# nsweb/dequan

Measured on NVIDIA B200. Metric: search_nodes_per_sec, higher is better.
Workload: dtype u32

## Files before the change

dequan_b200/csrc/dq_api.cu:

```cuda
#include <algorithm>
#include <condition_variable>
#include <cstdio>
#include <cstdlib>
#include <cstring>
#include <memory>
#include <mutex>
#include <string>
#include <thread>
#include <vector>

#include "dequan_b200.h"
#include "dq_kernels.cuh"
#include "dq_lane_queens.cuh"
#include "dq_lane_sudoku.cuh"
#include "dq_reg_graphs.cuh"
#include "dq_group_graphs.cuh"
#include "dq_small_tree.cuh"
#include "dq_lane_tree.cuh"
#include "dq_model.hpp"

namespace dq {

static thread_local std::string g_err;
void set_last_error(const std::string& s) { g_err = s; }
// ... 1135 lines not shown
}

static int run_batch_sudoku(dq_model* m, const uint8_t* cells_dev, int64_t n, int32_t stride, const dq_batch_opts* opts,
                            uint8_t* sol_dev, unsigned long long* nodes_dev, uint8_t* status_dev, dq_batch_stats* st) {
    int rc = DQ_OK;
    const unsigned long long task_cap = std::max<unsigned long long>(1u << 24, std::min<unsigned long long>(8ull * n, 1ull << 26));
    const unsigned long long snap_cap = std::min<unsigned long long>(std::max<unsigned long long>(1u << 20, (unsigned long long)n + (1u << 20)), 1ull << 24);
    const bool fresh_pool = m->s_tasks.cap < task_cap;
    DQ_CUDA(m->s_digest.reserve(n)); DQ_CUDA(m->s_hard.reserve(2 * (size_t)n)); DQ_CUDA(m->s_ctrl.reserve(16));
    DQ_CUDA(m->s_tasks.reserve(task_cap)); DQ_CUDA(m->s_snaps.reserve(snap_cap * kSnapWords)); DQ_CUDA(m->s_snap_state.reserve(snap_cap));
    unsigned long long* ctrl = m->s_ctrl.p;
    DQ_CUDA(cudaMemsetAsync(ctrl, 0, 16 * sizeof(unsigned long long), m->stream));
    DQ_CUDA(cudaMemsetAsync(m->s_snap_state.p, 0, snap_cap * sizeof(uint32_t), m->stream));
    const unsigned long long dirty = fresh_pool ? m->s_tasks.cap : std::min<unsigned long long>(m->s_tasks_used, m->s_tasks.cap);
    if (dirty) DQ_CUDA(cudaMemsetAsync(m->s_tasks.p, 0, dirty * sizeof(SudokuTask), m->stream));
    SudokuArgs A;
    A.digest = m->s_digest.p; A.n = n; A.stride = stride; A.cells = cells_dev; A.solution = sol_dev; A.nodes = nodes_dev;
    A.status = status_dev; A.hard = m->s_hard.p; A.tasks = m->s_tasks.p; A.task_cap = task_cap;
    A.snaps = m->s_snaps.p; A.snap_cap = snap_cap; A.snap_state = m->s_snap_state.p; A.ctrl = ctrl; A.user_budget = opts ? opts->node_budget : 0;
    A.force_donate = opts && opts->task_nodes > 0 ? (unsigned)opts->task_nodes : 0u;
    const char* env_dd = getenv("DQ_SUDOKU_DONATE_DEPTH");
    A.donate_depth = env_dd ? atoi(env_dd) : 5;
    const char* env_dm = getenv("DQ_SUDOKU_DONATE_MIN");
    const char* env_dg = getenv("DQ_SUDOKU_DONATE_GAP");
    A.donate_min = env_dm ? (unsigned)atoi(env_dm) : kDonateMinNodes;
    A.donate_gap = env_dg ? (unsigned)atoi(env_dg) : kDonateGap;
    const char* env_sg = getenv("DQ_SUDOKU_SPLIT_GAP");
    A.split_gap = env_sg ? (unsigned)atoi(env_sg) : kSplitGap;
    const char* env_h = getenv("DQ_SUDOKU_HIDDEN_AFTER");
    A.strong_hidden_after = env_h ? (unsigned)atoi(env_h) : kStrongHiddenAfter;
    const char* env_q = getenv("DQ_SUDOKU_POP_QUORUM");
    A.pop_quorum = env_q ? atoi(env_q) : kPopQuorum;
    const char* env_fb = getenv("DQ_SUDOKU_FIRST_BUDGET");
    A.first_budget = env_fb ? (unsigned)atoi(env_fb) : (n >= 400000 ? 3072u : 1024u);
    if (A.force_donate) A.first_budget = std::min(A.first_budget, 4u * A.force_donate);
    const bool trace = getenv("DQ_TRACE") != nullptr;
    cudaEvent_t ev[7] = {nullptr};
    if (trace) for (auto& e : ev) cudaEventCreate(&e);
    auto mark = [&](int i) { if (trace) cudaEventRecord(ev[i], m->stream); };
    const long long sms = m->sm_count;
    DQ_CUDA(cudaEventRecord(m->ev0, m->stream));
    mark(0);
    {
        int occ_d = 0;
        rc = max_ctas_per_sm(k_sudoku_digest, kDigestTile, kDigestSmem, &occ_d);
        if (rc != DQ_OK) return rc;
        const long long tiles = (n + kDigestTile - 1) / kDigestTile;
        k_sudoku_digest<<<(unsigned)std::max<long long>(1, std::min<long long>(tiles, (long long)std::max(occ_d, 1) * sms)), kDigestTile, kDigestSmem, m->stream>>>(
            cells_dev, n, stride, m->s_digest.p, ctrl + SKC_MAX_BLANK);
    }
    mark(1);
    unsigned long long* h_blank = m->pin + 117;
    DQ_CUDA(cudaMemcpyAsync(h_blank, ctrl + SKC_MAX_BLANK, sizeof(unsigned long long), cudaMemcpyDeviceToHost, m->stream));
    DQ_CUDA(cudaStreamSynchronize(m->stream));
    static const bool full_stack = getenv("DQ_SUDOKU_FULL_STACK") != nullptr;
    const int levels = full_stack ? 81 : (int)std::min<unsigned long long>(std::max<unsigned long long>(*h_blank, 1), 81);
    const size_t smem = offsetof(SudokuSmem, stk) + (size_t)levels * kSudokuBlock * sizeof(uint16_t);
    const size_t smem_strong = sudoku_strong_smem(levels);
    A.stack_levels = levels;
    int occ_first = 0, occ_count = 0, occ_walk = 0, occ_strong = 0;
    rc = max_ctas_per_sm(k_sudoku_first, kSudokuBlock, smem, &occ_first);
    if (rc == DQ_OK) rc = max_ctas_per_sm(k_sudoku_count, kSudokuBlock, smem, &occ_count);
    if (rc == DQ_OK) rc = max_ctas_per_sm(k_sudoku_walk, kSudokuBlock, smem, &occ_walk);
    if (rc == DQ_OK) rc = max_ctas_per_sm(k_sudoku_strong, 128, smem_strong, &occ_strong);
    if (rc != DQ_OK) return rc;
    if (occ_first < 1 || occ_count < 1 || occ_walk < 1 || occ_strong < 1) { g_err = "kernel does not fit an SM"; return DQ_ERR_UNSUPPORTED; }
    const long long ctas_first = std::max<long long>(1, std::min<long long>(occ_first * sms, (long long)((n + kSudokuBlock - 1) / kSudokuBlock)));
// ... 358 lines not shown
```

dequan_b200/csrc/dq_lane_sudoku.cuh:

```cuda
#pragma once
#include <cstdint>
#include <cuda_runtime.h>
#include "dq_group_graphs.cuh"

namespace dq {

constexpr int kSudokuBlock = 128;
constexpr uint32_t SK_ONES = 0x00100401u;
constexpr uint32_t SK_SPARE = 0x20080200u;
constexpr uint32_t SK_FULL3 = 0x1FF7FDFFu;
constexpr uint8_t SK_STATUS_HARD = 0xFD;
constexpr uint8_t SK_STATUS_DEFER = 0xFE;

constexpr int kDigestVec = 18;
constexpr int kTableWords = 63;
struct SudokuDigest { uint4 v[kDigestVec]; };

struct SudokuTask {
    uint32_t puzzle;
    uint32_t snap_id;
    uint32_t info;
    uint32_t pad;
};
constexpr uint32_t SKT_VALID = 0x80000000u, SKT_ROOT = 0x40000000u, SKT_NULL = 0x20000000u, SKT_TOP = 0x10000000u;
constexpr int kSnapWords = 12;

enum SkCtrl { SKC_FRESH = 0,
              SKC_HARD = 1,
              SKC_HARD_CUR = 2,
              SKC_WALK_CUR = 3,
              SKC_RESERVE = 4,
              SKC_SNAP = 5,
              SKC_HEAD = 6,
              SKC_OUTSTANDING = 7,
              SKC_MAX_BLANK = 8,
              SKC_ERROR = 9,
              SKC_TOTALS = 12 };

struct SudokuArgs {
    const SudokuDigest* digest;
    long long n;
    int stride;
    const uint8_t* cells;
    uint8_t* solution;
    unsigned long long* nodes;
    uint8_t* status;
    uint32_t* hard;
    SudokuTask* tasks;    unsigned long long task_cap;
    uint4* snaps;         unsigned long long snap_cap;
    uint32_t* snap_state;
    unsigned long long* ctrl;
    unsigned long long user_budget;
    unsigned first_budget;
    int donate_depth;
    unsigned donate_min, donate_gap;
    unsigned strong_hidden_after;
    int pop_quorum;
    int stack_levels;
    unsigned split_gap;
    unsigned force_donate;
};

constexpr int kDigestTile = 128;
constexpr int kDigestInBytes = kDigestTile * 81;
constexpr int kDigestOutBytes = kDigestTile * kDigestVec * 16;
constexpr int kDigestSmem = 2 * kDigestInBytes + kDigestOutBytes + 16;

__global__ void __launch_bounds__(kDigestTile)
k_sudoku_digest(const uint8_t* __restrict__ cells, long long n, int stride, SudokuDigest* __restrict__ out, unsigned long long* __restrict__ max_blank) {
    extern __shared__ __align__(128) uint8_t dg_raw[];
    uint8_t* recs = dg_raw + 2 * kDigestInBytes;
    const uint32_t in_s = smem_u32(dg_raw), recs_s = smem_u32(recs), mbar = recs_s + kDigestOutBytes;
    const long long tiles = (n + kDigestTile - 1) / kDigestTile;
    const bool bulk_ok = stride == 81 && ((size_t)cells & 15) == 0 && ((size_t)out & 15) == 0;
    if (threadIdx.x == 0) { mbar_init(mbar, 1); mbar_init(mbar + 8, 1); mbar_init_fence(); }
    __syncthreads();
    auto full = [&](long long t) { return bulk_ok && (t + 1) * kDigestTile <= n; };
    auto issue = [&](long long t, int b) {
        mbar_expect_tx(mbar + 8 * b, kDigestInBytes);
        bulk_g2s(in_s + b * kDigestInBytes, cells + t * kDigestInBytes, kDigestInBytes, mbar + 8 * b);
    };
    uint32_t parity = 0;
    int b = 0;
    int most_blanks = 0;
    long long t = blockIdx.x;
    if (t < tiles && full(t) && threadIdx.x == 0) issue(t, 0);
    bool store_in_flight = false;
    for (; t < tiles; t += gridDim.x, b ^= 1) {
        const long long nxt = t + gridDim.x;
        if (nxt < tiles && full(nxt) && threadIdx.x == 0) issue(nxt, b ^ 1);
        const long long first = t * kDigestTile;
        const int here = (int)min((long long)kDigestTile, n - first);
        uint8_t* stage = dg_raw + b * kDigestInBytes;
        if (full(t)) { mbar_wait(mbar + 8 * b, (parity >> b) & 1u); parity ^= 1u << b; }
// ... 6 lines not shown
            __syncthreads();
            store_in_flight = false;
        }
        if ((int)threadIdx.x < here) {
            const uint8_t* g = stage + threadIdx.x * 81;
            uint32_t row[9], col[9], box[9], blank[3] = {0, 0, 0};
#pragma unroll
            for (int i = 0; i < 9; i++) { row[i] = 0; col[i] = 0; box[i] = 0; }
            bool defer = false;
#pragma unroll
            for (int r = 0; r < 9; r++)
#pragma unroll
                for (int c = 0; c < 9; c++) {
                    const int p = r * 9 + c;
                    const uint32_t v = g[p];
                    if (v == 0) { blank[p >> 5] |= 1u << (p & 31); continue; }
                    if (v > 9) { defer = true; continue; }
                    const uint32_t bit = 1u << (v - 1);
                    const int bx = (r / 3) * 3 + c / 3;
                    if ((row[r] | col[c] | box[bx]) & bit) defer = true;
                    row[r] |= bit; col[c] |= bit; box[bx] |= bit;
                }
            uint32_t w[kDigestVec * 4];
#pragma unroll
            for (int i = 0; i < kDigestVec * 4; i++) w[i] = 0;
            int level = 0;
#pragma unroll
            for (int r = 0; r < 9; r++)
#pragma unroll
                for (int c = 0; c < 9; c++) {
                    const int p = r * 9 + c;
                    if (!((blank[p >> 5] >> (p & 31)) & 1u)) continue;
                    if ((row[r] | col[c] | box[(r / 3) * 3 + c / 3]) == 0x1FFu) defer = true;
                    w[19 + r * 3 + c / 3] |= 0x1FFu << (10 * (c % 3));
                    w[67 + (c * 9 + r) / 32] |= 1u << ((c * 9 + r) % 32);
                    ++level;
                }
            w[0] = blank[0]; w[1] = blank[1]; w[2] = blank[2];
            w[3] = (uint32_t)level | (defer ? 0x80000000u : 0u);
            most_blanks = max(most_blanks, level);
#pragma unroll
            for (int i = 0; i < 9; i++) w[10 + i] = box[i] * SK_ONES;
#pragma unroll
            for (int i = 0; i < 3; i++) {
                w[4 + i] = row[3 * i] | (row[3 * i + 1] << 10) | (row[3 * i + 2] << 20);
                w[7 + i] = col[3 * i] | (col[3 * i + 1] << 10) | (col[3 * i + 2] << 20);
            }
            uint32_t* rw = reinterpret_cast<uint32_t*>(recs + threadIdx.x * (kDigestVec * 16));
#pragma unroll
            for (int i = 0; i < kDigestVec * 4; i++) rw[i] = w[i];
            uint8_t* tab = recs + threadIdx.x * (kDigestVec * 16) + 46 * 4;
            int L = 0;
#pragma unroll
            for (int k = 0; k < 3; k++)
                for (uint32_t bits = blank[k]; bits; bits &= bits - 1u) tab[L++] = (uint8_t)(32 * k + __ffs((int)bits) - 1);
        }
        if (full(t)) {
            fence_async_smem();
            __syncthreads();
            if (threadIdx.x == 0) { bulk_s2g(out + first, recs_s, kDigestOutBytes); bulk_commit(); }
            store_in_flight = true;
        } else {
            __syncthreads();
            const uint4* src = reinterpret_cast<const uint4*>(recs);
            uint4* dst = reinterpret_cast<uint4*>(out + first);
            for (int i = threadIdx.x; i < here * kDigestVec; i += kDigestTile) dst[i] = src[i];
            __syncthreads();
        }
    }
    if (store_in_flight && threadIdx.x == 0) bulk_wait_read0();
    most_blanks = __reduce_max_sync(0xFFFFFFFFu, most_blanks);
    if ((threadIdx.x & 31) == 0 && most_blanks) atomicMax(max_blank, (unsigned long long)most_blanks);
}

struct SudokuSmem {
    uint32_t rowp[3][kSudokuBlock];
    uint32_t colp[3][kSudokuBlock];
    uint32_t boxr[9][kSudokuBlock];
    uint32_t blk[27][kSudokuBlock];
    uint32_t cellw[21][kSudokuBlock];
    uint16_t stk[81][kSudokuBlock];
};

__device__ __forceinline__ uint32_t sk_rep(uint32_t x9) { return x9 * SK_ONES; }

struct SkCell { int r, s, f, band, box, rm; };
__device__ __forceinline__ SkCell sk_decode(int p) {
    SkCell c;
    c.r = (p * 57) >> 9;
    const int col = p - 9 * c.r;
    c.s = (col * 11) >> 5;
    c.f = col - 3 * c.s;
    c.band = (c.r * 11) >> 5;
    c.box = c.band * 3 + c.s;
    c.rm = c.r - 3 * c.band;
    return c;
}

__device__ __forceinline__ uint32_t sk_singletons(uint32_t x) {
    const uint32_t y = x + (SK_SPARE - SK_ONES);
    const uint32_t z = x & y;
    const uint32_t tt = z + (SK_SPARE - SK_ONES);
    const uint32_t nz = ~tt & SK_SPARE;
    return x & (nz - (nz >> 9));
}

struct SkLane {
    bool have, enter;
    uint32_t puzzle;
    int p;
    SkCell c;
    int sp, base_sp, nblank;
    uint32_t passrem;
    uint32_t dom_rem;
    uint32_t nodes;
    unsigned long long nodes_hi;
};

__device__ __forceinline__ int sk_cell_at(const SudokuSmem& S, int t, int l) { return (int)((S.cellw[l >> 2][t] >> ((l & 3) * 8)) & 0xFF); }
__device__ __forceinline__ uint32_t sk_used_at(const SudokuSmem& S, int t, const SkCell& k) {
    return ((S.rowp[k.band][t] >> (10 * k.rm)) | (S.colp[k.s][t] >> (10 * k.f)) | S.boxr[k.box][t]) & 0x1FF;
}
__device__ __forceinline__ void sk_commit(SudokuSmem& S, int t, const SkCell& k, uint32_t bit) {
    S.rowp[k.band][t] |= bit << (10 * k.rm);
    S.boxr[k.box][t] |= sk_rep(bit);
    S.colp[k.s][t] |= bit << (10 * k.f);
}

__device__ __forceinline__ void sk_load_tables(SudokuSmem& S, int t, const uint4* __restrict__ dg) {
    uint32_t* dst = &S.rowp[0][t];
#pragma unroll
    for (int q = 1; q < kDigestVec; q++) {
        const uint4 x = __ldg(dg + q);
        const int wbase = 4 * q - 4;
        if (wbase + 0 < kTableWords) dst[(wbase + 0) * kSudokuBlock] = x.x;
        if (wbase + 1 < kTableWords) dst[(wbase + 1) * kSudokuBlock] = x.y;
        if (wbase + 2 < kTableWords) dst[(wbase + 2) * kSudokuBlock] = x.z;
        if (wbase + 3 < kTableWords) dst[(wbase + 3) * kSudokuBlock] = x.w;
    }
}
struct SkBlankT { uint32_t t0, t1, t2; };
__device__ __forceinline__ SkBlankT sk_load_blank_t(const uint4* __restrict__ dg) {
    const uint4 a = __ldg(dg + 16), b = __ldg(dg + 17);
    SkBlankT x; x.t0 = a.w; x.t1 = b.x; x.t2 = b.y;
    return x;
}

__device__ __forceinline__ void sk_enter(const SudokuSmem& S, int t, const SkCell& c, const SkBlankT& bt, uint32_t& dom, uint32_t& pass) {
    const uint32_t rowband = S.rowp[c.band][t];
    const uint32_t colw = S.colp[c.s][t];
    const uint32_t boxv = S.boxr[c.box][t];
    const uint32_t rowv = sk_rep((rowband >> (10 * c.rm)) & 0x1FF);
    const uint32_t colv = (colw >> (10 * c.f)) & 0x1FF;
    dom = ~(rowv | colv | boxv) & 0x1FF;
    uint32_t kill3 = sk_singletons(~(rowv | colw | boxv) & S.blk[c.r * 3 + c.s][t] & (0xFFFFFFFFu << (10 * c.f + 10)) & SK_FULL3);
    {
        const uint32_t* colp = &S.colp[c.s][t];
        const uint32_t* boxp = &S.boxr[c.box][t];
        const uint32_t* blkp = &S.blk[c.r * 3 + c.s][t];
#pragma unroll
        for (int k = 1; k <= 2; k++) {
            const bool on = c.s + k < 3;
            const uint32_t u = on ? (rowv | colp[k * kSudokuBlock] | boxp[k * kSudokuBlock]) : 0xFFFFFFFFu;
            const uint32_t b = on ? blkp[k * kSudokuBlock] : 0u;
            kill3 |= sk_singletons(~u & b);
        }
    }
    {
        const uint32_t* blkp = &S.blk[c.r * 3 + c.s][t];
#pragma unroll
        for (int k = 1; k <= 2; k++) {
            const bool on = c.rm + k < 3;
            const uint32_t rv = sk_rep((rowband >> (on ? 10 * (c.rm + k) : 0)) & 0x1FF);
            const uint32_t b = on ? blkp[3 * k * kSudokuBlock] : 0u;
            kill3 |= sk_singletons(~(rv | colw | boxv) & b);
        }
    }
    {
        const uint32_t crep = sk_rep(colv);
        const uint32_t* rowp = &S.rowp[c.band][t];
        const uint32_t* boxp = &S.boxr[c.box][t];
        const int q0 = 9 * (3 * c.s + c.f) + 3 * c.band;
#pragma unroll
        for (int k = 1; k <= 2; k++) {
            const bool on = c.band + k < 3;
            const int q = q0 + 3 * k;
            const uint32_t lo = q < 32 ? bt.t0 : (q < 64 ? bt.t1 : bt.t2);
            const uint32_t hi = q < 32 ? bt.t1 : (q < 64 ? bt.t2 : 0u);
            const uint32_t m3 = on ? (__funnelshift_r(lo, hi, q & 31) & 7u) : 0u;
            const uint32_t b = ((m3 * 0x00040201u) & SK_ONES) * 0x1FFu;
            const uint32_t u = on ? (crep | rowp[k * kSudokuBlock] | boxp[3 * k * kSudokuBlock]) : 0xFFFFFFFFu;
            kill3 |= sk_singletons(~u & b);
        }
    }
    const uint32_t kill = (kill3 | (kill3 >> 10) | (kill3 >> 20)) & 0x1FF;
    pass = dom & ~kill;
}

__device__ __forceinline__ bool sk_pop(SudokuSmem& S, int t, SkLane& L) {
    L.nodes += __popc(L.dom_rem);
    if (L.sp == L.base_sp) return true;
    --L.sp;
    const uint32_t e = S.stk[L.sp][t];
    const uint32_t v = e >> 9, bit = 1u << v;
    L.p = sk_cell_at(S, t, L.sp);
    L.c = sk_decode(L.p);
    S.rowp[L.c.band][t] ^= bit << (10 * L.c.rm);
    S.boxr[L.c.box][t] ^= sk_rep(bit);
    S.colp[L.c.s][t] ^= bit << (10 * L.c.f);
    L.passrem = e & 0x1FF;
    L.dom_rem = ~sk_used_at(S, t, L.c) & 0x1FF & ~((2u << v) - 1u);
    return false;
}

__device__ __forceinline__ bool sk_choose(SudokuSmem& S, int t, SkLane& L) {
    const uint32_t nxt = L.passrem & (0u - L.passrem);
    L.nodes += __popc(L.dom_rem & (nxt | (nxt - 1u)));
    L.passrem ^= nxt;
    const uint32_t v = __ffs(nxt) - 1;
    S.stk[L.sp][t] = (uint16_t)(L.passrem | (v << 9));
    if (L.sp == L.nblank - 1) return true;
    sk_commit(S, t, L.c, nxt);
    ++L.sp;
    L.p = sk_cell_at(S, t, L.sp);
    L.enter = true;
    return false;
}

__device__ __forceinline__ uint32_t sk_snap_entry(const uint4* __restrict__ sb, int l) {
    const uint4 cur = __ldcg(sb + (l >> 3));
    const uint32_t word = (l & 4) ? ((l & 2) ? cur.w : cur.z) : ((l & 2) ? cur.y : cur.x);
    return (l & 1) ? (word >> 16) : (word & 0xFFFF);
}
__device__ __forceinline__ void sk_snap_write(uint4* __restrict__ sb, const SudokuSmem& S, int t, int upto, uint32_t extra0, uint32_t extra1) {
    for (int q = 0; q * 8 <= upto + 1; q++) {
        uint32_t w4[4];
#pragma unroll
        for (int i = 0; i < 4; i++) {
            const int l0 = q * 8 + 2 * i, l1 = l0 + 1;
            const uint32_t e0 = l0 < upto ? (uint32_t)S.stk[l0][t] : (l0 == upto ? extra0 : (l0 == upto + 1 ? extra1 : 0u));
            const uint32_t e1 = l1 < upto ? (uint32_t)S.stk[l1][t] : (l1 == upto ? extra0 : (l1 == upto + 1 ? extra1 : 0u));
            w4[i] = e0 | (e1 << 16);
        }
        __stcg(sb + q, make_uint4(w4[0], w4[1], w4[2], w4[3]));
    }
}

constexpr int kPopQuorum = 10;

__device__ __forceinline__ void sk_store_solutions(const SudokuSmem& S, const SudokuArgs& A, int t, bool fin, uint32_t puzzle,
                                                   uint32_t b0, uint32_t b1, uint32_t b2) {
    const int lane = t & 31;
    const uint32_t lt = (1u << lane) - 1u;
    __syncwarp();
    uint32_t fm = __ballot_sync(0xFFFFFFFFu, fin);
    while (fm) {
        const int Ls = __ffs(fm) - 1;
        fm &= fm - 1;
        const uint32_t x0 = __shfl_sync(0xFFFFFFFFu, b0, Ls), x1 = __shfl_sync(0xFFFFFFFFu, b1, Ls), x2 = __shfl_sync(0xFFFFFFFFu, b2, Ls);
        const uint32_t pz = __shfl_sync(0xFFFFFFFFu, puzzle, Ls);
        uint8_t* out = A.solution + (size_t)pz * A.stride;
        const uint8_t* in = A.cells + (size_t)pz * A.stride;
        const int tL = (t & ~31) + Ls;
#pragma unroll
        for (int k = 0; k < 3; k++) {
            const int cell = lane + 32 * k;
            if (cell < 81) {
                const uint32_t bw = k == 0 ? x0 : (k == 1 ? x1 : x2);
                uint8_t val;
                if ((bw >> lane) & 1u) {
                    const int level = __popc(bw & lt) + (k > 0 ? __popc(x0) : 0) + (k > 1 ? __popc(x1) : 0);
                    val = (uint8_t)((S.stk[level][tL] >> 9) + 1);
                } else val = in[cell];
                out[cell] = val;
            }
        }
    }
}

__global__ void __launch_bounds__(kSudokuBlock)
k_sudoku_first(SudokuArgs A) {
    extern __shared__ __align__(16) unsigned char sk_raw[];
    SudokuSmem& S = *reinterpret_cast<SudokuSmem*>(sk_raw);
    const int t = threadIdx.x;
    const int lane = t & 31;
    const uint32_t lt = (1u << lane) - 1u;
    const unsigned long long total_warps = (unsigned long long)gridDim.x * (kSudokuBlock / 32);

    SkLane L = {};
    SkBlankT bt = {0, 0, 0};
    uint32_t b0 = 0, b1 = 0, b2 = 0;
    uint32_t limit = 0;
    bool limit_is_api = false, done = false;
    unsigned long long chunk_pos = 0, chunk_end = 0;
    bool exhausted = false;

    for (;;) {
        const uint32_t need = __ballot_sync(0xFFFFFFFFu, !L.have && !done);
        if (need) {
            const uint32_t n_need = __popc(need);
            if (chunk_pos >= chunk_end && !exhausted) {
                unsigned long long base = 0;
                uint32_t size = 0;
                if (lane == 0) {
                    const unsigned long long cur = *(volatile unsigned long long*)(A.ctrl + SKC_FRESH);
                    const unsigned long long remaining = cur < (unsigned long long)A.n ? (unsigned long long)A.n - cur : 0;
                    size = (uint32_t)min(max(remaining / (8ull * total_warps), (unsigned long long)n_need), 64ull);
                    base = atomicAdd(A.ctrl + SKC_FRESH, (unsigned long long)size);
                }
                base = __shfl_sync(0xFFFFFFFFu, base, 0);
                size = __shfl_sync(0xFFFFFFFFu, size, 0);
                chunk_pos = base;
                chunk_end = min(base + size, (unsigned long long)A.n);
                if (base >= (unsigned long long)A.n) { exhausted = true; chunk_end = chunk_pos; }
            }
            const unsigned long long avail = chunk_end - chunk_pos;
            if (!L.have && !done) {
                const uint32_t rank = __popc(need & lt);
                if (rank < avail) {
                    L.puzzle = (uint32_t)(chunk_pos + rank);
                    const uint4* dg = A.digest[L.puzzle].v;
                    const uint4 head = __ldg(dg);
                    b0 = head.x; b1 = head.y; b2 = head.z;
                    L.nblank = (int)(head.w & 0xFF);
                    L.nodes = 0; L.nodes_hi = 0;
                    limit = A.first_budget; limit_is_api = false;
                    bool skip = false;
                    if (head.w & 0x80000000u) { A.status[L.puzzle] = SK_STATUS_DEFER; skip = true; }
                    else if (A.user_budget) {
                        const unsigned long long givens = 81 - L.nblank;
                        if (A.user_budget < givens) {
                            A.nodes[L.puzzle] = A.user_budget + 1; A.status[L.puzzle] = 2; skip = true;
                            uint8_t* out = A.solution + (size_t)L.puzzle * A.stride;
                            for (int i = 0; i < 81; i++) out[i] = 0;
                        } else if (A.user_budget - givens + 1 <= (unsigned long long)limit) {
                            limit = (uint32_t)(A.user_budget - givens + 1);
                            limit_is_api = true;
                        }
                    }
                    if (!skip && L.nblank == 0) {
                        A.nodes[L.puzzle] = 81; A.status[L.puzzle] = 1;
                        uint8_t* out = A.solution + (size_t)L.puzzle * A.stride;
                        const uint8_t* in = A.cells + (size_t)L.puzzle * A.stride;
                        for (int i = 0; i < 81; i++) out[i] = in[i];
                        skip = true;
                    }
                    if (!skip) {
                        sk_load_tables(S, t, dg);
                        bt = sk_load_blank_t(dg);
                        L.sp = 0; L.base_sp = 0; L.passrem = 0; L.dom_rem = 0;
                        L.p = sk_cell_at(S, t, 0);
                        L.enter = true;
                        L.have = true;
                    }
                } else if (exhausted) done = true;
            }
            chunk_pos += min((unsigned long long)n_need, avail);
            if (__all_sync(0xFFFFFFFFu, done && !L.have)) break;
        }

        for (int rep = 0;; rep++) {
            const bool popping = L.have && !L.enter && L.passrem == 0;
            const uint32_t pm = __ballot_sync(0xFFFFFFFFu, popping);
            if (pm == 0 || (rep > 0 && __popc(pm) < A.pop_quorum)) break;
            if (popping && sk_pop(S, t, L)) {
                A.nodes[L.puzzle] = (81 - L.nblank) + L.nodes_hi + L.nodes;
                A.status[L.puzzle] = 0;
                uint8_t* out = A.solution + (size_t)L.puzzle * A.stride;
                for (int i = 0; i < 81; i++) out[i] = 0;
                L.have = false;
            }
        }

        bool fin = false;
        if (L.have && !L.enter && L.passrem != 0 && sk_choose(S, t, L)) {
            A.nodes[L.puzzle] = (81 - L.nblank) + L.nodes_hi + L.nodes;
            A.status[L.puzzle] = 1;
            fin = true;
            L.have = false;
        }

        if (L.have && L.enter) {
            L.c = sk_decode(L.p);
            uint32_t dom, pass;
            sk_enter(S, t, L.c, bt, dom, pass);
            L.dom_rem = dom; L.passrem = pass; L.enter = false;
        }

        if (L.have && L.nodes >= limit) {
            if (limit_is_api) {
                A.nodes[L.puzzle] = A.user_budget + 1; A.status[L.puzzle] = 2;
                uint8_t* out = A.solution + (size_t)L.puzzle * A.stride;
                for (int i = 0; i < 81; i++) out[i] = 0;
            } else {
                const unsigned long long sslot = atomicAdd(A.ctrl + SKC_SNAP, 1ull);
                const unsigned long long idx = atomicAdd(A.ctrl + SKC_HARD, 1ull);
                if (sslot < A.snap_cap) { sk_snap_write(A.snaps + (size_t)sslot * kSnapWords, S, t, L.sp, L.passrem, L.dom_rem); A.snap_state[sslot] = 1u; }
                else atomicOr(A.ctrl + SKC_ERROR, 2ull);
                A.hard[2 * idx] = L.puzzle;
                A.hard[2 * idx + 1] = (uint32_t)sslot | ((uint32_t)L.sp << 24);
                A.nodes[L.puzzle] = (81 - L.nblank) + L.nodes_hi + L.nodes;
                A.status[L.puzzle] = SK_STATUS_HARD;
            }
            L.have = false;
        }

        sk_store_solutions(S, A, t, fin, L.puzzle, b0, b1, b2);
    }
}

constexpr unsigned kStrongHiddenAfter = 400;

struct StrongSmem {
    uint32_t peer[81][32];
};
__host__ __device__ inline size_t sudoku_strong_smem(int levels) { return sizeof(StrongSmem) + (size_t)4 * levels * (32 * 4 + 2) + 16; }

__device__ __forceinline__ bool sk_hidden_singles(uint32_t& D, int lane, uint32_t u0, uint32_t u1, uint32_t u2, bool& changed) {
// ... 58 lines not shown
    uint16_t* const rest = reinterpret_cast<uint16_t*>(sk_raw + sizeof(StrongSmem) + (size_t)4 * A.stack_levels * 128) + wib * A.stack_levels;
    for (int i = threadIdx.x; i < 81 * 32; i += blockDim.x) {
        const int x = i >> 5, l = i & 31;
        const int xr = x / 9, xc = x % 9;
        uint32_t m = 0;
        for (int f = 0; f < 3; f++) {
            const int q = l + 32 * f;
            if (q >= 81 || q == x) continue;
            const int qr = q / 9, qc = q % 9;
            if (qr == xr || qc == xc || (qr / 3 == xr / 3 && qc / 3 == xc / 3)) m |= 1u << (10 * f);
        }
        M.peer[x][l] = m;
    }
    __syncthreads();
    const uint32_t valid3 = lane < 17 ? SK_ONES : 0x00000401u;
    uint32_t u0 = 0, u1 = 0, u2 = 0;
    if (lane < 27)
        for (int k = 0; k < 9; k++) {
            const int cell = lane < 9 ? lane * 9 + k : (lane < 18 ? k * 9 + (lane - 9)
                                                                  : ((lane - 18) / 3 * 3 + k / 3) * 9 + ((lane - 18) % 3 * 3 + k % 3));
            const uint32_t bit = 1u << (cell & 31);
            if (cell < 32) u0 |= bit; else if (cell < 64) u1 |= bit; else u2 |= bit;
        }
    const unsigned long long n_hard = A.ctrl[SKC_HARD];
    for (;;) {
        unsigned long long idx = 0;
        if (lane == 0) idx = atomicAdd(A.ctrl + SKC_HARD_CUR, 1ull);
        idx = __shfl_sync(0xFFFFFFFFu, idx, 0);
        if (idx >= n_hard) break;
        const uint32_t puzzle = A.hard[2 * idx];
        const uint8_t* in = A.cells + (size_t)puzzle * A.stride;
        const uint32_t* dw = reinterpret_cast<const uint32_t*>(A.digest[puzzle].v);
        const int nblank = (int)(__ldg(dw + 3) & 0xFF);
        const uint32_t cw = lane < 21 ? __ldg(dw + 46 + lane) : 0u;
        uint32_t D = 0;
#pragma unroll
        for (int f = 0; f < 3; f++) {
            const int q = lane + 32 * f;
            if (q < 81) {
                const uint32_t g = in[q];
                uint32_t field;
                if (g) field = (1u << (g - 1)) | 0x200u;
                else {
                    const SkCell k = sk_decode(q);
                    field = ~((__ldg(dw + 4 + k.band) >> (10 * k.rm)) | (__ldg(dw + 7 + k.s) >> (10 * k.f)) | __ldg(dw + 10 + k.box)) & 0x1FF;
                }
                D |= field << (10 * f);
            }
        }
        unsigned tries = 0;
        int l = sk_propagate(D, M, lane, valid3, false, u0, u1, u2) ? 0 : -1;
        bool back = false;
        while (l >= 0 && l < nblank) {
            const int p = (int)((__shfl_sync(0xFFFFFFFFu, cw, l >> 2) >> ((l & 3) * 8)) & 0xFF);
            const int owner = p & 31, f = p >> 5;
            uint32_t d;
            if (!back) {
                const uint32_t w = __shfl_sync(0xFFFFFFFFu, D, owner) >> (10 * f);
                if (w & 0x200u) {
                    if (lane == 0) rest[l] = 0;
                    __syncwarp();
                    ++l;
                    continue;
                }
                d = w & 0x1FF;
                saved[l * 32] = D;
            } else d = rest[l];
            bool ok = false;
            while (d) {
                const uint32_t v = d & (0u - d);
                d ^= v;
                D = saved[l * 32];
                if (lane == owner) D = (D & ~(0x3FFu << (10 * f))) | ((v | 0x200u) << (10 * f));
                D &= ~(M.peer[p][lane] * v);
                ++tries;
                if (sk_propagate(D, M, lane, valid3, tries > A.strong_hidden_after, u0, u1, u2)) { ok = true; break; }
            }
            __syncwarp();
            if (lane == 0) rest[l] = (uint16_t)d;
            __syncwarp();
            if (ok) { ++l; back = false; }
            else {
                --l;
                while (l >= 0 && rest[l] == 0) --l;
                back = true;
            }
        }
// ... 5 lines not shown
            if (q < 81) out[q] = sat ? (uint8_t)__ffs((D >> (10 * f)) & 0x1FF) : (uint8_t)0;
        }
        if (lane == 0) A.status[puzzle] = sat ? 1 : 0;
        __syncwarp();
    }
}

__global__ void __launch_bounds__(kSudokuBlock)
k_sudoku_walk(SudokuArgs A) {
    extern __shared__ __align__(16) unsigned char sk_raw[];
    SudokuSmem& S = *reinterpret_cast<SudokuSmem*>(sk_raw);
    const int t = threadIdx.x;
    const int lane = t & 31;
    const unsigned long long n_hard = A.ctrl[SKC_HARD];
    auto emit = [&](uint32_t puzzle, uint32_t snap, uint32_t info) {
        const unsigned long long slot = atomicAdd(A.ctrl + SKC_RESERVE, 1ull);
        if (slot >= A.task_cap) { atomicOr(A.ctrl + SKC_ERROR, 2ull); return; }
        atomicAdd(A.ctrl + SKC_OUTSTANDING, 1ull);
        *reinterpret_cast<uint4*>(A.tasks + slot) = make_uint4(puzzle, snap, SKT_VALID | info, 0u);
    };
    for (;;) {
        unsigned long long base = 0;
        if (lane == 0) base = atomicAdd(A.ctrl + SKC_WALK_CUR, 32ull);
        base = __shfl_sync(0xFFFFFFFFu, base, 0);
        if (base >= n_hard) break;
        const bool active = base + lane < n_hard;
        const uint32_t puzzle = active ? A.hard[2 * (base + lane)] : 0u;
        const uint32_t hinfo = active ? A.hard[2 * (base + lane) + 1] : 0u;
        const uint32_t snap = hinfo & 0xFFFFFFu;
        const int psp = (int)(hinfo >> 24);
        const uint4* sb = A.snaps + (size_t)snap * kSnapWords;
        int nblank = 0;
        bool sat = false;
        SkBlankT bt = {0, 0, 0};
        if (active) {
            const uint4* dg = A.digest[puzzle].v;
            nblank = (int)(__ldg(dg).w & 0xFF);
            sk_load_tables(S, t, dg);
            bt = sk_load_blank_t(dg);
            sat = A.status[puzzle] == 1;
        }
        const uint8_t* sol = A.solution + (size_t)puzzle * A.stride;
        if (active && !sat) emit(puzzle, snap, SKT_TOP | 0u | ((uint32_t)psp << 8));
        unsigned long long direct = 0;
        bool on_parked_path = true;
        const int levels = active && sat ? nblank : 0;
        const int max_levels = __reduce_max_sync(0xFFFFFFFFu, levels);
        for (int l = 0; l < max_levels; l++) {
            if (l < levels) {
                const int p = sk_cell_at(S, t, l);
                const SkCell c = sk_decode(p);
                const uint32_t bit = 1u << (sol[p] - 1);
                uint32_t dom_rem, passrem;
                bool charge = true;
                if (on_parked_path && l < psp) {
                    const uint32_t e = sk_snap_entry(sb, l);
                    const uint32_t v = e >> 9;
                    if ((1u << v) == bit) charge = false;
                    else {
                        if ((1u << v) > bit) atomicOr(A.ctrl + SKC_ERROR, 8ull);
                        emit(puzzle, snap, SKT_TOP | (uint32_t)(l + 1) | ((uint32_t)psp << 8));
                        passrem = e & 0x1FF;
                        dom_rem = ~sk_used_at(S, t, c) & 0x1FF & ~((2u << v) - 1u);
                        on_parked_path = false;
                    }
                } else if (on_parked_path && l == psp) {
                    passrem = sk_snap_entry(sb, l) & 0x1FF;
                    dom_rem = sk_snap_entry(sb, l + 1) & 0x1FF;
                    on_parked_path = false;
                } else {
                    uint32_t dom, pass;
                    sk_enter(S, t, c, bt, dom, pass);
                    dom_rem = dom; passrem = pass;
                }
                if (charge) {
                    direct += __popc(dom_rem & (bit | (bit - 1u)));
                    if (!(passrem & bit)) atomicOr(A.ctrl + SKC_ERROR, 8ull);
                    uint32_t V = passrem & (bit - 1u);
                    while (V) {
                        const uint32_t v = __ffs(V) - 1;
                        V &= V - 1;
                        emit(puzzle, 0u, SKT_ROOT | (uint32_t)l | (v << 8));
                    }
                }
                sk_commit(S, t, c, bit);
            }
        }
        if (active && direct) atomicAdd(A.nodes + puzzle, direct);
    }
}

constexpr int kDonatePeriod = 32;
constexpr uint32_t kDonateMinNodes = 48;
constexpr uint32_t kDonateGap = 96;
constexpr uint32_t kSplitGap = 512;

__global__ void __launch_bounds__(kSudokuBlock)
k_sudoku_count(SudokuArgs A) {
    extern __shared__ __align__(16) unsigned char sk_raw[];
    SudokuSmem& S = *reinterpret_cast<SudokuSmem*>(sk_raw);
    const int t = threadIdx.x;
    const int lane = t & 31;
    const uint32_t lt = (1u << lane) - 1u;
    const unsigned long long total_warps = (unsigned long long)gridDim.x * (kSudokuBlock / 32);
    volatile unsigned long long* vctrl = A.ctrl;

    SkLane L = {};
    SkBlankT bt = {0, 0, 0};
    uint32_t donate_at = 0;
    uint32_t split_at = 0;
    bool waiting = false, poll_now = false;
    unsigned long long ticket = 0;
    int iter = 0;
    unsigned spins = 0;

    for (;;) {
        {
            const uint32_t need = __ballot_sync(0xFFFFFFFFu, !L.have && !waiting);
            if (need) {
                unsigned long long base = 0;
                if (lane == 0) base = atomicAdd(A.ctrl + SKC_HEAD, (unsigned long long)__popc(need));
                base = __shfl_sync(0xFFFFFFFFu, base, 0);
                if (!L.have && !waiting) { ticket = base + __popc(need & lt); waiting = true; poll_now = true; }
            }
        }
        unsigned closed_now = 0;
        uint32_t got_info = 0, got_snap = 0;
        if (waiting && (poll_now || (iter & 7) == 0) && ticket < A.task_cap) {
            volatile uint32_t* rec = reinterpret_cast<volatile uint32_t*>(A.tasks + ticket);
            const uint32_t info = rec[2];
            if (info) {
                __threadfence();
                waiting = false;
                L.puzzle = rec[0];
                if (info & SKT_NULL) closed_now = 1;
                else { got_info = info; got_snap = rec[1]; }
            }
        }
        for (uint32_t todo = __ballot_sync(0xFFFFFFFFu, got_info != 0u); todo; todo &= todo - 1u) {
            const int src = __ffs((int)todo) - 1;
            const uint32_t pz = __shfl_sync(0xFFFFFFFFu, L.puzzle, src), inf = __shfl_sync(0xFFFFFFFFu, got_info, src);
            const uint32_t sn = __shfl_sync(0xFFFFFFFFu, got_snap, src);
            const int ts = (t & ~31) + src;
            const uint32_t* dgw = reinterpret_cast<const uint32_t*>(A.digest[pz].v);
            uint32_t* tab = &S.rowp[0][0];
            for (int w = lane; w < kTableWords; w += 32) tab[w * kSudokuBlock + ts] = __ldg(dgw + 4 + w);
            __syncwarp();
            const bool root = (inf & SKT_ROOT) != 0u;
            const int lo = (int)(inf & 0xFF), hi = (int)((inf >> 8) & 0xFF);
            const int n_replay = root ? lo + 1 : hi;
            const uint8_t* sol = A.solution + (size_t)pz * A.stride;
            const uint4* sb = A.snaps + (size_t)sn * kSnapWords;
            for (int l = lane; l < n_replay; l += 32) {
                const int q = sk_cell_at(S, ts, l);
                uint32_t v, entry;
                if (root) { v = l < lo ? (uint32_t)sol[q] - 1u : (uint32_t)(hi & 0xF); entry = v << 9; }
                else { const uint32_t e = sk_snap_entry(sb, l); v = e >> 9; entry = l >= lo ? e : (e & 0xFE00u); }
                const SkCell k = sk_decode(q);
                const uint32_t bit = 1u << v;
                atomicOr(&S.rowp[k.band][ts], bit << (10 * k.rm));
                atomicOr(&S.boxr[k.box][ts], sk_rep(bit));
                atomicOr(&S.colp[k.s][ts], bit << (10 * k.f));
                S.stk[l][ts] = (uint16_t)entry;
            }
            __syncwarp();
        }
        if (got_info) {
            const uint32_t info = got_info;
            const uint4* dg = A.digest[L.puzzle].v;
            L.nblank = (int)(__ldg(dg).w & 0xFF);
            bt = sk_load_blank_t(dg);
            L.nodes = 0; L.nodes_hi = 0;
            L.passrem = 0; L.dom_rem = 0;
            L.have = true;
            donate_at = A.force_donate ? A.force_donate : A.donate_min;
            split_at = A.split_gap;
            if (info & SKT_ROOT) {
                const int l0 = (int)(info & 0xFF);
                L.sp = l0 + 1; L.base_sp = l0 + 1;
                if (L.sp >= L.nblank) { atomicOr(A.ctrl + SKC_ERROR, 4ull); L.have = false; closed_now = 1; }
                else { L.p = sk_cell_at(S, t, L.sp); L.enter = true; }
            } else {
                const int lo = (int)(info & 0xFF), hi = (int)((info >> 8) & 0xFF);
                const uint4* sb = A.snaps + (size_t)got_snap * kSnapWords;
                L.sp = hi; L.base_sp = lo;
                L.p = sk_cell_at(S, t, hi);
                L.c = sk_decode(L.p);
                const uint32_t e = sk_snap_entry(sb, hi);
                L.passrem = e & 0x1FF;
                if (info & SKT_TOP) L.dom_rem = sk_snap_entry(sb, hi + 1) & 0x1FF;
                else L.dom_rem = ~sk_used_at(S, t, L.c) & 0x1FF & ~((2u << (e >> 9)) - 1u);
                L.enter = false;
                __threadfence();
                A.snap_state[got_snap] = 0u;
            }
        }
        poll_now = false;
        {
            const uint32_t cm = __ballot_sync(0xFFFFFFFFu, closed_now != 0);
            if (cm && lane == 0) atomicAdd(A.ctrl + SKC_OUTSTANDING, 0ull - (unsigned long long)__popc(cm));
            if (cm) continue;
        }
        if (__ballot_sync(0xFFFFFFFFu, L.have) == 0) {
            unsigned long long out = 0;
            if (lane == 0) out = vctrl[SKC_OUTSTANDING];
            out = __shfl_sync(0xFFFFFFFFu, out, 0);
            if (out == 0) break;
            __nanosleep(spins < 4096u ? 200u : 2000u);
            if (++spins > 120000000u) { if (lane == 0) atomicOr(A.ctrl + SKC_ERROR, 1ull); break; }
            poll_now = true;
            continue;
        }
        spins = 0;
        ++iter;

        if ((iter & (kDonatePeriod - 1)) == 0) {
            long long demand = 0;
            if (lane == 0) {
                const unsigned long long h = vctrl[SKC_HEAD], r = vctrl[SKC_RESERVE];
                demand = h > r ? (long long)(h - r) : 0;
// ... 22 lines not shown
                            atomicAdd(A.ctrl + SKC_OUTSTANDING, 0ull - 1ull);
                            A.snap_state[sslot] = 0u;
                            donate_at = 0xFFFFFFFFu; split_at = 0xFFFFFFFFu;
                        } else {
                            sk_snap_write(A.snaps + (size_t)sslot * kSnapWords, S, t, hl + 1, 0u, 0u);
                            volatile uint32_t* rec = reinterpret_cast<volatile uint32_t*>(A.tasks + slot);
                            rec[0] = L.puzzle; rec[1] = (uint32_t)sslot;
                            __threadfence();
                            rec[2] = SKT_VALID | (uint32_t)L.base_sp | ((uint32_t)hl << 8);
                            L.base_sp = hl + 1;
                            donate_at = L.nodes + (A.force_donate ? A.force_donate : A.donate_gap);
                            split_at = L.nodes + A.split_gap;
                        }
                    }
                }
            }
        }

        unsigned closed = 0;
        for (int rep = 0;; rep++) {
            const bool popping = L.have && !L.enter && L.passrem == 0;
            const uint32_t pm = __ballot_sync(0xFFFFFFFFu, popping);
            if (pm == 0 || (rep > 0 && __popc(pm) < A.pop_quorum)) break;
            if (popping && sk_pop(S, t, L)) {
                atomicAdd(A.nodes + L.puzzle, L.nodes_hi + L.nodes);
                L.have = false; closed = 1;
            }
        }

        if (L.have && !L.enter && L.passrem != 0 && sk_choose(S, t, L))
            atomicOr(A.ctrl + SKC_ERROR, 4ull);

        if (L.have && L.enter) {
            L.c = sk_decode(L.p);
            uint32_t dom, pass;
            sk_enter(S, t, L.c, bt, dom, pass);
            L.dom_rem = dom; L.passrem = pass; L.enter = false;
        }
        if (L.nodes >= 0x80000000u) { L.nodes_hi += L.nodes; L.nodes = 0; donate_at = 0; split_at = A.split_gap; }

        {
            const uint32_t cm = __ballot_sync(0xFFFFFFFFu, closed != 0);
            if (cm && lane == 0) atomicAdd(A.ctrl + SKC_OUTSTANDING, 0ull - (unsigned long long)__popc(cm));
        }
    }
}

__global__ void k_sudoku_finish(SudokuArgs A, unsigned long long* totals) {
    const long long i = (long long)blockIdx.x * blockDim.x + threadIdx.x;
    unsigned sat = 0, unsat = 0, budget = 0;
    unsigned long long nd = 0;
    if (i < A.n) {
        uint8_t st = A.status[i];
        if (st != SK_STATUS_DEFER) {
            if (A.user_budget && A.nodes[i] > A.user_budget && st != 2) {
                st = 2;
                A.nodes[i] = A.user_budget + 1;
                uint8_t* out = A.solution + (size_t)i * A.stride;
                for (int c = 0; c < 81; c++) out[c] = 0;
            }
            A.status[i] = st;
            nd = A.nodes[i];
            sat = st == 1; unsat = st == 0; budget = st == 2;
        }
    }
    for (int o = 16; o > 0; o >>= 1) {
        sat += __shfl_down_sync(0xFFFFFFFFu, sat, o);
        unsat += __shfl_down_sync(0xFFFFFFFFu, unsat, o);
        budget += __shfl_down_sync(0xFFFFFFFFu, budget, o);
// ... 18 lines not shown
```

Baseline: 565.1 billion.

## Compact sudoku digest: replace per-cell blank masks with bit masks and packed cell descriptors

Shrinks the per-puzzle digest from 18 to 12 uint4 words. The 27 shared-memory blank-mask words are replaced by compact row-major and column-major blank bitmaps kept in registers, and the cell order table now stores pre-decoded band/row/stack/column descriptors instead of raw cell indices. This removes the sk_decode arithmetic, a large block of shared memory per thread, and digest bandwidth, which should raise occupancy and lower memory traffic. The cost is some extra shift and select logic in sk_enter. The first-task node budget for large batches is also lowered from 3072 to 2048.

```diff
diff --git a/dequan_b200/csrc/dq_api.cu b/dequan_b200/csrc/dq_api.cu
--- a/dequan_b200/csrc/dq_api.cu
+++ b/dequan_b200/csrc/dq_api.cu
@@ -1191,7 +1191,7 @@
     const char* env_q = getenv("DQ_SUDOKU_POP_QUORUM");
     A.pop_quorum = env_q ? atoi(env_q) : kPopQuorum;
     const char* env_fb = getenv("DQ_SUDOKU_FIRST_BUDGET");
-    A.first_budget = env_fb ? (unsigned)atoi(env_fb) : (n >= 400000 ? 3072u : 1024u);
+    A.first_budget = env_fb ? (unsigned)atoi(env_fb) : (n >= 400000 ? 2048u : 1024u);
     if (A.force_donate) A.first_budget = std::min(A.first_budget, 4u * A.force_donate);
     const bool trace = getenv("DQ_TRACE") != nullptr;
     cudaEvent_t ev[7] = {nullptr};
diff --git a/dequan_b200/csrc/dq_lane_sudoku.cuh b/dequan_b200/csrc/dq_lane_sudoku.cuh
--- a/dequan_b200/csrc/dq_lane_sudoku.cuh
+++ b/dequan_b200/csrc/dq_lane_sudoku.cuh
@@ -12,8 +12,8 @@
 constexpr uint8_t SK_STATUS_HARD = 0xFD;
 constexpr uint8_t SK_STATUS_DEFER = 0xFE;
 
-constexpr int kDigestVec = 18;
-constexpr int kTableWords = 63;
+constexpr int kDigestVec = 12;
+constexpr int kTableWords = 36;
 struct SudokuDigest { uint4 v[kDigestVec]; };
 
 struct SudokuTask {
@@ -60,6 +60,30 @@
     unsigned split_gap;
     unsigned force_donate;
 };
+
+struct SkCell { int s, f, band, box, rm; };
+__host__ __device__ __forceinline__ SkCell sk_decode(int p) {
+    SkCell c;
+    const int r = (p * 57) >> 9;
+    const int col = p - 9 * r;
+    c.s = (col * 11) >> 5;
+    c.f = col - 3 * c.s;
+    c.band = (r * 11) >> 5;
+    c.box = c.band * 3 + c.s;
+    c.rm = r - 3 * c.band;
+    return c;
+}
+__host__ __device__ __forceinline__ uint32_t sk_desc(int p) {
+    const SkCell c = sk_decode(p);
+    return (uint32_t)(c.band | c.rm << 2 | c.s << 4 | c.f << 6);
+}
+__device__ __forceinline__ SkCell sk_unpack(uint32_t d) {
+    SkCell c;
+    c.band = d & 3; c.rm = (d >> 2) & 3; c.s = (d >> 4) & 3; c.f = d >> 6;
+    c.box = c.band * 3 + c.s;
+    return c;
+}
+__device__ __forceinline__ int sk_desc_cell(uint32_t d) { return 27 * (d & 3) + 9 * ((d >> 2) & 3) + 3 * ((d >> 4) & 3) + (d >> 6); }
 
 constexpr int kDigestTile = 128;
 constexpr int kDigestInBytes = kDigestTile * 81;
@@ -132,8 +156,8 @@
                     const int p = r * 9 + c;
                     if (!((blank[p >> 5] >> (p & 31)) & 1u)) continue;
                     if ((row[r] | col[c] | box[(r / 3) * 3 + c / 3]) == 0x1FFu) defer = true;
-                    w[19 + r * 3 + c / 3] |= 0x1FFu << (10 * (c % 3));
-                    w[67 + (c * 9 + r) / 32] |= 1u << ((c * 9 + r) % 32);
+                    w[40 + r / 3] |= 1u << (10 * (c % 3) + 3 * (r % 3) + c / 3);
+                    w[44 + c / 3] |= 1u << (10 * (r % 3) + 3 * (c % 3) + r / 3);
                     ++level;
                 }
             w[0] = blank[0]; w[1] = blank[1]; w[2] = blank[2];
@@ -149,11 +173,11 @@
             uint32_t* rw = reinterpret_cast<uint32_t*>(recs + threadIdx.x * (kDigestVec * 16));
 #pragma unroll
             for (int i = 0; i < kDigestVec * 4; i++) rw[i] = w[i];
-            uint8_t* tab = recs + threadIdx.x * (kDigestVec * 16) + 46 * 4;
+            uint8_t* tab = recs + threadIdx.x * (kDigestVec * 16) + 19 * 4;
             int L = 0;
 #pragma unroll
             for (int k = 0; k < 3; k++)
-                for (uint32_t bits = blank[k]; bits; bits &= bits - 1u) tab[L++] = (uint8_t)(32 * k + __ffs((int)bits) - 1);
+                for (uint32_t bits = blank[k]; bits; bits &= bits - 1u) tab[L++] = (uint8_t)sk_desc(32 * k + __ffs((int)bits) - 1);
         }
         if (full(t)) {
             fence_async_smem();
@@ -177,25 +201,11 @@
     uint32_t rowp[3][kSudokuBlock];
     uint32_t colp[3][kSudokuBlock];
     uint32_t boxr[9][kSudokuBlock];
-    uint32_t blk[27][kSudokuBlock];
-    uint32_t cellw[21][kSudokuBlock];
+    uint32_t lvl[21][kSudokuBlock];
     uint16_t stk[81][kSudokuBlock];
 };
 
 __device__ __forceinline__ uint32_t sk_rep(uint32_t x9) { return x9 * SK_ONES; }
-
-struct SkCell { int r, s, f, band, box, rm; };
-__device__ __forceinline__ SkCell sk_decode(int p) {
-    SkCell c;
-    c.r = (p * 57) >> 9;
-    const int col = p - 9 * c.r;
-    c.s = (col * 11) >> 5;
-    c.f = col - 3 * c.s;
-    c.band = (c.r * 11) >> 5;
-    c.box = c.band * 3 + c.s;
-    c.rm = c.r - 3 * c.band;
-    return c;
-}
 
 __device__ __forceinline__ uint32_t sk_singletons(uint32_t x) {
     const uint32_t y = x + (SK_SPARE - SK_ONES);
@@ -205,10 +215,17 @@
     return x & (nz - (nz >> 9));
 }
 
+__device__ __forceinline__ uint32_t sk_singletons_at(uint32_t x, uint32_t blank) {
+    const uint32_t y = x + (SK_SPARE - SK_ONES);
+    const uint32_t z = x & y;
+    const uint32_t tt = z + (SK_SPARE - SK_ONES);
+    const uint32_t one = ~(tt >> 9) & blank & SK_ONES;
+    return x & (one * 0x1FFu);
+}
+
 struct SkLane {
     bool have, enter;
     uint32_t puzzle;
-    int p;
     SkCell c;
     int sp, base_sp, nblank;
     uint32_t passrem;
@@ -217,7 +234,7 @@
     unsigned long long nodes_hi;
 };
 
-__device__ __forceinline__ int sk_cell_at(const SudokuSmem& S, int t, int l) { return (int)((S.cellw[l >> 2][t] >> ((l & 3) * 8)) & 0xFF); }
+__device__ __forceinline__ uint32_t sk_desc_at(const SudokuSmem& S, int t, int l) { return (S.lvl[l >> 2][t] >> ((l & 3) * 8)) & 0xFF; }
 __device__ __forceinline__ uint32_t sk_used_at(const SudokuSmem& S, int t, const SkCell& k) {
     return ((S.rowp[k.band][t] >> (10 * k.rm)) | (S.colp[k.s][t] >> (10 * k.f)) | S.boxr[k.box][t]) & 0x1FF;
 }
@@ -239,58 +256,51 @@
         if (wbase + 3 < kTableWords) dst[(wbase + 3) * kSudokuBlock] = x.w;
     }
 }
-struct SkBlankT { uint32_t t0, t1, t2; };
-__device__ __forceinline__ SkBlankT sk_load_blank_t(const uint4* __restrict__ dg) {
-    const uint4 a = __ldg(dg + 16), b = __ldg(dg + 17);
-    SkBlankT x; x.t0 = a.w; x.t1 = b.x; x.t2 = b.y;
+struct SkBlank { uint32_t w0, w1, w2, t0, t1, t2; };
+__device__ __forceinline__ SkBlank sk_load_blank(const uint4* __restrict__ dg) {
+    const uint4 a = __ldg(dg + 10), b = __ldg(dg + 11);
+    SkBlank x; x.w0 = a.x; x.w1 = a.y; x.w2 = a.z; x.t0 = b.x; x.t1 = b.y; x.t2 = b.z;
     return x;
 }
 
-__device__ __forceinline__ void sk_enter(const SudokuSmem& S, int t, const SkCell& c, const SkBlankT& bt, uint32_t& dom, uint32_t& pass) {
+__device__ __forceinline__ void sk_enter(const SudokuSmem& S, int t, const SkCell& c, const SkBlank& bl, uint32_t& dom, uint32_t& pass) {
     const uint32_t rowband = S.rowp[c.band][t];
     const uint32_t colw = S.colp[c.s][t];
     const uint32_t boxv = S.boxr[c.box][t];
     const uint32_t rowv = sk_rep((rowband >> (10 * c.rm)) & 0x1FF);
     const uint32_t colv = (colw >> (10 * c.f)) & 0x1FF;
     dom = ~(rowv | colv | boxv) & 0x1FF;
-    uint32_t kill3 = sk_singletons(~(rowv | colw | boxv) & S.blk[c.r * 3 + c.s][t] & (0xFFFFFFFFu << (10 * c.f + 10)) & SK_FULL3);
+    const uint32_t xb = (c.band == 0 ? bl.w0 : (c.band == 1 ? bl.w1 : bl.w2)) >> (3 * c.rm + c.s);
+    uint32_t kill3 = sk_singletons_at(~(rowv | colw | boxv) & (0xFFFFFFFFu << (10 * c.f + 10)) & SK_FULL3, xb);
     {
         const uint32_t* colp = &S.colp[c.s][t];
         const uint32_t* boxp = &S.boxr[c.box][t];
-        const uint32_t* blkp = &S.blk[c.r * 3 + c.s][t];
 #pragma unroll
         for (int k = 1; k <= 2; k++) {
             const bool on = c.s + k < 3;
             const uint32_t u = on ? (rowv | colp[k * kSudokuBlock] | boxp[k * kSudokuBlock]) : 0xFFFFFFFFu;
-            const uint32_t b = on ? blkp[k * kSudokuBlock] : 0u;
-            kill3 |= sk_singletons(~u & b);
+            kill3 |= sk_singletons_at(~u & SK_FULL3, xb >> k);
         }
     }
     {
-        const uint32_t* blkp = &S.blk[c.r * 3 + c.s][t];
 #pragma unroll
         for (int k = 1; k <= 2; k++) {
             const bool on = c.rm + k < 3;
             const uint32_t rv = sk_rep((rowband >> (on ? 10 * (c.rm + k) : 0)) & 0x1FF);
-            const uint32_t b = on ? blkp[3 * k * kSudokuBlock] : 0u;
-            kill3 |= sk_singletons(~(rv | colw | boxv) & b);
+            const uint32_t u = on ? (rv | colw | boxv) : 0xFFFFFFFFu;
+            kill3 |= sk_singletons_at(~u & SK_FULL3, xb >> (3 * k));
         }
     }
     {
         const uint32_t crep = sk_rep(colv);
         const uint32_t* rowp = &S.rowp[c.band][t];
         const uint32_t* boxp = &S.boxr[c.box][t];
-        const int q0 = 9 * (3 * c.s + c.f) + 3 * c.band;
+        const uint32_t xs = (c.s == 0 ? bl.t0 : (c.s == 1 ? bl.t1 : bl.t2)) >> (3 * c.f + c.band);
 #pragma unroll
         for (int k = 1; k <= 2; k++) {
             const bool on = c.band + k < 3;
-            const int q = q0 + 3 * k;
-            const uint32_t lo = q < 32 ? bt.t0 : (q < 64 ? bt.t1 : bt.t2);
-            const uint32_t hi = q < 32 ? bt.t1 : (q < 64 ? bt.t2 : 0u);
-            const uint32_t m3 = on ? (__funnelshift_r(lo, hi, q & 31) & 7u) : 0u;
-            const uint32_t b = ((m3 * 0x00040201u) & SK_ONES) * 0x1FFu;
             const uint32_t u = on ? (crep | rowp[k * kSudokuBlock] | boxp[3 * k * kSudokuBlock]) : 0xFFFFFFFFu;
-            kill3 |= sk_singletons(~u & b);
+            kill3 |= sk_singletons_at(~u & SK_FULL3, xs >> k);
         }
     }
     const uint32_t kill = (kill3 | (kill3 >> 10) | (kill3 >> 20)) & 0x1FF;
@@ -303,8 +313,7 @@
     --L.sp;
     const uint32_t e = S.stk[L.sp][t];
     const uint32_t v = e >> 9, bit = 1u << v;
-    L.p = sk_cell_at(S, t, L.sp);
-    L.c = sk_decode(L.p);
+    L.c = sk_unpack(sk_desc_at(S, t, L.sp));
     S.rowp[L.c.band][t] ^= bit << (10 * L.c.rm);
     S.boxr[L.c.box][t] ^= sk_rep(bit);
     S.colp[L.c.s][t] ^= bit << (10 * L.c.f);
@@ -322,7 +331,7 @@
     if (L.sp == L.nblank - 1) return true;
     sk_commit(S, t, L.c, nxt);
     ++L.sp;
-    L.p = sk_cell_at(S, t, L.sp);
+    L.c = sk_unpack(sk_desc_at(S, t, L.sp));
     L.enter = true;
     return false;
 }
@@ -388,7 +397,7 @@
     const unsigned long long total_warps = (unsigned long long)gridDim.x * (kSudokuBlock / 32);
 
     SkLane L = {};
-    SkBlankT bt = {0, 0, 0};
+    SkBlank bl = {0, 0, 0, 0, 0, 0};
     uint32_t b0 = 0, b1 = 0, b2 = 0;
     uint32_t limit = 0;
     bool limit_is_api = false, done = false;
@@ -447,9 +456,9 @@
                     }
                     if (!skip) {
                         sk_load_tables(S, t, dg);
-                        bt = sk_load_blank_t(dg);
+                        bl = sk_load_blank(dg);
                         L.sp = 0; L.base_sp = 0; L.passrem = 0; L.dom_rem = 0;
-                        L.p = sk_cell_at(S, t, 0);
+                        L.c = sk_unpack(sk_desc_at(S, t, 0));
                         L.enter = true;
                         L.have = true;
                     }
@@ -481,9 +490,8 @@
         }
 
         if (L.have && L.enter) {
-            L.c = sk_decode(L.p);
             uint32_t dom, pass;
-            sk_enter(S, t, L.c, bt, dom, pass);
+            sk_enter(S, t, L.c, bl, dom, pass);
             L.dom_rem = dom; L.passrem = pass; L.enter = false;
         }
 
@@ -608,7 +616,7 @@
         const uint8_t* in = A.cells + (size_t)puzzle * A.stride;
         const uint32_t* dw = reinterpret_cast<const uint32_t*>(A.digest[puzzle].v);
         const int nblank = (int)(__ldg(dw + 3) & 0xFF);
-        const uint32_t cw = lane < 21 ? __ldg(dw + 46 + lane) : 0u;
+        const uint32_t cw = lane < 21 ? __ldg(dw + 19 + lane) : 0u;
         uint32_t D = 0;
 #pragma unroll
         for (int f = 0; f < 3; f++) {
@@ -628,7 +636,7 @@
         int l = sk_propagate(D, M, lane, valid3, false, u0, u1, u2) ? 0 : -1;
         bool back = false;
         while (l >= 0 && l < nblank) {
-            const int p = (int)((__shfl_sync(0xFFFFFFFFu, cw, l >> 2) >> ((l & 3) * 8)) & 0xFF);
+            const int p = sk_desc_cell((__shfl_sync(0xFFFFFFFFu, cw, l >> 2) >> ((l & 3) * 8)) & 0xFF);
             const int owner = p & 31, f = p >> 5;
             uint32_t d;
             if (!back) {
@@ -700,12 +708,12 @@
         const uint4* sb = A.snaps + (size_t)snap * kSnapWords;
         int nblank = 0;
         bool sat = false;
-        SkBlankT bt = {0, 0, 0};
+        SkBlank bl = {0, 0, 0, 0, 0, 0};
         if (active) {
             const uint4* dg = A.digest[puzzle].v;
             nblank = (int)(__ldg(dg).w & 0xFF);
             sk_load_tables(S, t, dg);
-            bt = sk_load_blank_t(dg);
+            bl = sk_load_blank(dg);
             sat = A.status[puzzle] == 1;
         }
         const uint8_t* sol = A.solution + (size_t)puzzle * A.stride;
@@ -716,9 +724,9 @@
         const int max_levels = __reduce_max_sync(0xFFFFFFFFu, levels);
         for (int l = 0; l < max_levels; l++) {
             if (l < levels) {
-                const int p = sk_cell_at(S, t, l);
-                const SkCell c = sk_decode(p);
-                const uint32_t bit = 1u << (sol[p] - 1);
+                const uint32_t d = sk_desc_at(S, t, l);
+                const SkCell c = sk_unpack(d);
+                const uint32_t bit = 1u << (sol[sk_desc_cell(d)] - 1);
                 uint32_t dom_rem, passrem;
                 bool charge = true;
                 if (on_parked_path && l < psp) {
@@ -738,7 +746,7 @@
                     on_parked_path = false;
                 } else {
                     uint32_t dom, pass;
-                    sk_enter(S, t, c, bt, dom, pass);
+                    sk_enter(S, t, c, bl, dom, pass);
                     dom_rem = dom; passrem = pass;
                 }
                 if (charge) {
@@ -774,7 +782,7 @@
     volatile unsigned long long* vctrl = A.ctrl;
 
     SkLane L = {};
-    SkBlankT bt = {0, 0, 0};
+    SkBlank bl = {0, 0, 0, 0, 0, 0};
     uint32_t donate_at = 0;
     uint32_t split_at = 0;
     bool waiting = false, poll_now = false;
@@ -820,11 +828,11 @@
             const uint8_t* sol = A.solution + (size_t)pz * A.stride;
             const uint4* sb = A.snaps + (size_t)sn * kSnapWords;
             for (int l = lane; l < n_replay; l += 32) {
-                const int q = sk_cell_at(S, ts, l);
+                const uint32_t d = sk_desc_at(S, ts, l);
                 uint32_t v, entry;
-                if (root) { v = l < lo ? (uint32_t)sol[q] - 1u : (uint32_t)(hi & 0xF); entry = v << 9; }
+                if (root) { v = l < lo ? (uint32_t)sol[sk_desc_cell(d)] - 1u : (uint32_t)(hi & 0xF); entry = v << 9; }
                 else { const uint32_t e = sk_snap_entry(sb, l); v = e >> 9; entry = l >= lo ? e : (e & 0xFE00u); }
-                const SkCell k = sk_decode(q);
+                const SkCell k = sk_unpack(d);
                 const uint32_t bit = 1u << v;
                 atomicOr(&S.rowp[k.band][ts], bit << (10 * k.rm));
                 atomicOr(&S.boxr[k.box][ts], sk_rep(bit));
@@ -837,7 +845,7 @@
             const uint32_t info = got_info;
             const uint4* dg = A.digest[L.puzzle].v;
             L.nblank = (int)(__ldg(dg).w & 0xFF);
-            bt = sk_load_blank_t(dg);
+            bl = sk_load_blank(dg);
             L.nodes = 0; L.nodes_hi = 0;
             L.passrem = 0; L.dom_rem = 0;
             L.have = true;
@@ -847,13 +855,12 @@
                 const int l0 = (int)(info & 0xFF);
                 L.sp = l0 + 1; L.base_sp = l0 + 1;
                 if (L.sp >= L.nblank) { atomicOr(A.ctrl + SKC_ERROR, 4ull); L.have = false; closed_now = 1; }
-                else { L.p = sk_cell_at(S, t, L.sp); L.enter = true; }
+                else { L.c = sk_unpack(sk_desc_at(S, t, L.sp)); L.enter = true; }
             } else {
                 const int lo = (int)(info & 0xFF), hi = (int)((info >> 8) & 0xFF);
                 const uint4* sb = A.snaps + (size_t)got_snap * kSnapWords;
                 L.sp = hi; L.base_sp = lo;
-                L.p = sk_cell_at(S, t, hi);
-                L.c = sk_decode(L.p);
+                L.c = sk_unpack(sk_desc_at(S, t, hi));
                 const uint32_t e = sk_snap_entry(sb, hi);
                 L.passrem = e & 0x1FF;
                 if (info & SKT_TOP) L.dom_rem = sk_snap_entry(sb, hi + 1) & 0x1FF;
@@ -942,9 +949,8 @@
             atomicOr(A.ctrl + SKC_ERROR, 4ull);
 
         if (L.have && L.enter) {
-            L.c = sk_decode(L.p);
             uint32_t dom, pass;
-            sk_enter(S, t, L.c, bt, dom, pass);
+            sk_enter(S, t, L.c, bl, dom, pass);
             L.dom_rem = dom; L.passrem = pass; L.enter = false;
         }
         if (L.nodes >= 0x80000000u) { L.nodes_hi += L.nodes; L.nodes = 0; donate_at = 0; split_at = A.split_gap; }
```

Measured after the change: 565.1 billion (median of 6 runs). About the same (+0.0%).
